# BenCooper305/RL-Cattle-Herding

Measured on AMD Instinct MI355X. Metric: env-steps/sec (agent-steps/sec) at 4096 envs/GPU, 1/2/4/8 MI355X, higher is better.
Workload: dtype f64; 1 GPU; BASELINE configs[3]: 4096 envs/GPU x (4 drones, 16 cattle), CTDE obs (12,86), random-action rollout with auto-reset; envs_per_gpu=4096, num_drones=4, num_cattle=16, mode=ctde, physics=pyb, parallelism=env-sharded x1 (no per-step collective)

## Files before the change

### rl-cattle-herding_amd/csrc/ch_api.cpp

```cpp
#include <hip/hip_runtime.h>

#include <algorithm>
#include <cstdlib>
#include <cmath>
#include <cstdio>
#include <cstring>
#include <new>
#include <string>
#include <vector>

#include "ch_handle.h"
#include "ch_spawn_table.inc"

using namespace ch;

thread_local std::string g_create_err;

static const double kEpisodeLen[8] = {40, 40, 40, 40, 80, 40, 80, 80};
static const int kLevelMin[8] = {3, 4, 4, 4, 4, 4, 4, 4};
static const int kLevelMax[8] = {3, 4, 4, 4, 4, 4, 12, 12};

static uint64_t splitmix(uint64_t& s) {
    uint64_t z = (s += 0x9E3779B97F4A7C15ull);
    z = (z ^ (z >> 30)) * 0xBF58476D1CE4E5B9ull;
// ... 657 lines not shown
}

int ch__set_geometry(ch_handle* h, int32_t G, int32_t block) {
    if (!h || G < 1 || G > 64 || G * h->NC > 64 || block < 128 || block % 64 ||
        block > ((h->pw || h->cfg.physics != CH_PHYS_PYB) ? CH_V2_MAX_BLOCK_PW : CH_V2_MAX_BLOCK))
        return CH_ERR_INVALID;
    if (G * h->M > 3 * (block - 64)) return CH_ERR_UNSUPPORTED;
    size_t lds = V2Layout(G, h->NC, h->M, h->P, h->cfg.mode, (int)h->rsize, h->pw ? block / 64 - 1 : 0).bytes();
    if (lds > 160 * 1024) return CH_ERR_UNSUPPORTED;
    bool sep = false;
    if (!h->pw) {
        const size_t l = V2Layout(G, h->NC, h->M, h->P, h->cfg.mode, (int)h->rsize, 0, true).bytes();
        if (l <= 160 * 1024) { sep = true; lds = l; }
    }
    h->G = G; h->block = block; h->lds = lds; h->sep = sep;
    HIP_TRY(h, prepare_step(h));
    return CH_OK;
}

int ch__geometry(const ch_handle* h, int32_t* G, int32_t* block, int64_t* lds, int32_t* kernel) {
    if (!h) return CH_ERR_INVALID;
    if (G) *G = h->G;
    if (block) *block = h->block;
    if (lds) *lds = (int64_t)h->lds;
    if (kernel) *kernel = h->kernel;
    return CH_OK;
}

int ch__obs_invalidate(ch_handle* h, void* stream) {
    if (!h) return CH_ERR_INVALID;
    h->obs_zero_ptr = nullptr;
    HIP_TRY(h, hipSetDevice(h->device));
    HIP_TRY(h, hipMemsetAsync(h->stale + h->E, 1, (size_t)h->E, (hipStream_t)stream));
    return CH_OK;
}

int ch__set_phase_mask(ch_handle* h, int32_t mask) {
    if (!h) return CH_ERR_INVALID;
    h->phase_mask = mask;
    return CH_OK;
}

int ch_metrics(ch_handle* h, double* out, int32_t reset_after, void* stream) {
    if (!h || !out) return fail(h, CH_ERR_INVALID, "ch_metrics: NULL argument");
    HIP_TRY(h, hipSetDevice(h->device));
    hipStream_t st = (hipStream_t)stream;
    HIP_TRY(h, launch_metrics_reduce(h->metrics, h->E, h->mdev, h->errw, h->mdev + CH_METRIC_COUNT, reset_after, st));
    HIP_TRY(h, hipMemcpyAsync(h->mhost, h->mdev, sizeof(double) * (CH_METRIC_COUNT + 1), hipMemcpyDeviceToHost, st));
    HIP_TRY(h, hipStreamSynchronize(st));
    std::memcpy(out, h->mhost, sizeof(double) * CH_METRIC_COUNT);
    return device_status(h, (int)h->mhost[CH_METRIC_COUNT]);
}

int ch_metrics_device(ch_handle* h, double* dev_out, int32_t reset_after, void* stream) {
    if (!h || !dev_out) return fail(h, CH_ERR_INVALID, "ch_metrics_device: NULL argument");
    HIP_TRY(h, hipSetDevice(h->device));
    HIP_TRY(h, launch_metrics_reduce(h->metrics, h->E, dev_out, nullptr, nullptr, reset_after, (hipStream_t)stream));
    return CH_OK;
}

int ch_get_eval(ch_handle* h, double* host_out, void* stream) {
    if (!h || !host_out) return fail(h, CH_ERR_INVALID, "ch_get_eval: NULL argument");
    if (!h->evald) return fail(h, CH_ERR_UNSUPPORTED, "ch_get_eval: the handle was created with eval_metrics = 0");
    HIP_TRY(h, hipSetDevice(h->device));
    HIP_TRY(h, hipStreamSynchronize((hipStream_t)stream));
    HIP_TRY(h, hipMemcpy(host_out, h->evald, sizeof(double) * h->E * h->NC, hipMemcpyDeviceToHost));
    return CH_OK;
}

int ch_outputs_to_host(ch_handle* h, const ch_step_io* io, ch_host_out* out, void* stream) {
    if (!h) return fail(nullptr, CH_ERR_INVALID, "ch_outputs_to_host: NULL handle");
    if (!io || !out || !io->obs || !io->reward || !io->terminated || !io->truncated || !out->obs || !out->reward ||
        !out->terminated || !out->truncated)
        return fail(h, CH_ERR_INVALID, "ch_outputs_to_host: obs, reward, terminated and truncated are required on both sides");
    if ((out->reset_happened || out->ended_env || out->ended_obs || out->ended_stats) && !io->reset_happened)
        return fail(h, CH_ERR_INVALID, "ch_outputs_to_host: the reset list needs io->reset_happened");
    if ((out->ended_obs && !io->terminal_obs) || (out->ended_stats && !io->episode_stats))
        return fail(h, CH_ERR_INVALID, "ch_outputs_to_host: ended_obs needs io->terminal_obs, ended_stats io->episode_stats");
    if (out->agent_active && !io->agent_active)
        return fail(h, CH_ERR_INVALID, "ch_outputs_to_host: agent_active needs io->agent_active");
    HIP_TRY(h, hipSetDevice(h->device));
    hipStream_t st = (hipStream_t)stream;
    const int64_t E = h->E;
    const size_t blk = (size_t)h->rows * 86, live = (size_t)h->NC * 86;
    if (io->reset_happened) {
        if (!h->st.count) {
            HIP_TRY(h, hipMalloc(&h->st.count, sizeof(long long)));
            HIP_TRY(h, hipMalloc(&h->st.env, sizeof(long long) * E));
            HIP_TRY(h, hipMalloc(&h->st.stats, sizeof(double) * 2 * E));
            HIP_TRY(h, hipMalloc(&h->st.obs, sizeof(float) * blk * E));
            HIP_TRY(h, hipHostMalloc(&h->st.count_host, sizeof(long long), hipHostMallocDefault));
        }
        HIP_TRY(h, launch_stage_ended(E, io->reset_happened, out->ended_obs ? io->terminal_obs : nullptr,
                                      out->ended_stats ? io->episode_stats : nullptr, (int)blk, h->st.count, h->st.env,
                                      h->st.stats, h->st.obs, st));
        HIP_TRY(h, hipMemcpyAsync(h->st.count_host, h->st.count, sizeof(long long), hipMemcpyDeviceToHost, st));
    }
    if (live == blk)
        HIP_TRY(h, hipMemcpyAsync(out->obs, io->obs, sizeof(float) * blk * E, hipMemcpyDeviceToHost, st));
    else
        HIP_TRY(h, hipMemcpy2DAsync(out->obs, sizeof(float) * blk, io->obs, sizeof(float) * blk, sizeof(float) * live, E,
                                    hipMemcpyDeviceToHost, st));
    const size_t K = (size_t)h->K;
    HIP_TRY(h, hipMemcpyAsync(out->reward, io->reward, sizeof(float) * K * E, hipMemcpyDeviceToHost, st));
    HIP_TRY(h, hipMemcpyAsync(out->terminated, io->terminated, K * E, hipMemcpyDeviceToHost, st));
    HIP_TRY(h, hipMemcpyAsync(out->truncated, io->truncated, K * E, hipMemcpyDeviceToHost, st));
// ... 42 lines not shown
```

### rl-cattle-herding_amd/csrc/ch_step_body.h

```cpp
#pragma once
#include <hip/hip_runtime.h>

#include <atomic>

#include "ch_common.h"
#include "ch_device.h"
#include "ch_internal.h"

namespace ch {

enum { I_N = 0, I_SC, I_SCA, I_HASPREV, I_LEVEL, I_TALLY, I_SPAWN, I_ACTIVE, I_EPISODE, I_FLOCK, I_RESET, I_NEWN,
       I_HERD, I_OBSD, I_COUNT };
static_assert(I_COUNT == kV2EnvInts, "LDS env-int rows");
enum { F_D = 0, F_T, F_H, F_A, F_E, F_R, F_X0, F_X1, F_X2,
       C_PAIRS, C_ROWS, C_COWS, C_FLOCK, C_DELTA, F_W, F_Q,
       Q_LEN, C_QUEUE, F_C,
       C_EULER,
       V_DSIMD,
       F_RSV0, F_RSV1, F_RSV2,
       F_HC,
       FLAG_COUNT };
static_assert(FLAG_COUNT <= kV2Flags, "LDS flag words");
#define FL_LIST (I_COUNT * G)
#define RS_LIST (I_COUNT * G + G)
// ... 538 lines not shown
    const R C2B = R(2 * 4.47213595499958);
    R gx = 0, gy = 0, cxx = 0, cyy = 0, sx = 0, sy = 0;
    int nb = 0;
    constexpr int NK = NT ? NT : 64;
    CH_UNROLL for (int k = 0; k < NK; ++k) {
        if (k >= N || k >= n) break;
        R t[6];
        const int f = delta_vals(S, N, u, g, k, t);
        if (f & 1) { ++nb; gx += t[0]; gy += t[1]; cxx += t[2]; cyy += t[3]; }
        if (f & 2) { sx += t[4]; sy += t[5]; }
    }
    ddx = 0; ddy = 0;
    if (nb > 0) { ddx = C2B * gx + C2B * cxx; ddy = C2B * gy + C2B * cyy; }
    ddx += sx; ddy += sy;
}

template <class R>
__device__ __forceinline__ void velocity_update(const StepParams<R>& p, const V2Smem<R>& S, int M, int e0, int u, R ddx,
                                                R ddy, R* nv = nullptr, int GM = 0) {
    const long long CS = (long long)p.E * M;
    const R C1G = R(5), C2G = R(0.2 * 2.23606797749979);
    const R qix = S.cx[u], qiy = S.cy[u], pix = S.cvx[u], piy = S.cvy[u];
    R gmx = -C1G * sigma_1(qix - R(1)) - C2G * pix, gmy = -C1G * sigma_1(qiy - R(1)) - C2G * piy;
    R qx = (S.aux[u] + ddx) + gmx, qy = (S.auy[u] + ddy) + gmy;
    const R dt_sqr = R(0.05 * 0.05);
    R vx = pix + qx * dt_sqr, vy = piy + qy * dt_sqr;
    R sp = norm2(vx, vy);
    if (sp > R(kMaxVelCattle)) { R f = R(kMaxVelCattle) / sp; vx *= f; vy *= f; }
    if (nv) { nv[u] = vx; nv[GM + u] = vy; return; }
    const long long ci = (long long)e0 * M + u;
    CH_STS(&p.cattle[2 * CS + ci], vx); CH_STS(&p.cattle[3 * CS + ci], vy);
}

template <class R>
__device__ __forceinline__ void flock_combine(const StepParams<R>& p, V2Smem<R>& S, int N, int M, int e0, int u, int n,
                                              const R* td, const uint8_t* tdf, int ib, int T) {
    const R C2B = R(2 * 4.47213595499958);
    R ddx = 0, ddy = 0, sx = 0, sy = 0, gx = 0, gy = 0, cxx = 0, cyy = 0;
    int nb = 0;
    CH_UNROLL for (int k = 0; k < N; ++k) {
        if (k >= n) break;
        const int i = ib + k;
        const int f = tdf[i];
        if (f & 1) { ++nb; gx += td[i]; gy += td[T + i]; cxx += td[2 * T + i]; cyy += td[3 * T + i]; }
        if (f & 2) { sx += td[4 * T + i]; sy += td[5 * T + i]; }
    }
    if (nb > 0) { ddx = C2B * gx + C2B * cxx; ddy = C2B * gy + C2B * cyy; }
    ddx += sx; ddy += sy;
    velocity_update(p, S, M, e0, u, ddx, ddy);
}

template <class R>
struct V2Pipe {
    enum { P_N = 0, P_B, P_C, P_SIMD, P_COUNT = 8 };
    static constexpr size_t kBytes = (27 + 7) * 64 * sizeof(R) + (2 * 64 + kV2Flags + P_COUNT) * sizeof(int);
    R *ho, *d1;
    int *hoi, *flags1, *sync;
    __device__ explicit V2Pipe(unsigned char* base) {
        ho = (R*)base; d1 = ho + 27 * 64;
        hoi = (int*)(d1 + 7 * 64); flags1 = hoi + 2 * 64; sync = flags1 + kV2Flags;
    }
};

template <class R, int MODE, int GT, int NT, int MT, bool PHYS, bool PW, bool TOBS, int ROLE = 0>
__device__ __forceinline__ void step2_body(const StepParams<R>& p, int salt = 0, int kstep = 0) {
    extern __shared__ __align__(16) unsigned char smem_[];
    unsigned char* const smem = smem_ + salt;
    constexpr bool PIPE = ROLE != 0;
    static_assert(!PIPE || (sizeof(R) == 8 && MODE == 0 && GT == 16 && NT == 4 && !PW && !TOBS && !PHYS),
                  "the pipelined step loop is the configs[3] f64 instantiation's");
    constexpr bool marl = MODE == 1;
    constexpr bool MIX = sizeof(R) == 4;
    using PT = double;
    constexpr bool QUAD = !marl && GT == 16 && NT == 4;
    const int G = GT ? GT : p.G, N = NT ? NT : p.NC, M = MT ? MT : p.M, P = MT ? MT * (MT - 1) / 2 : p.P;
    const int rows = marl ? N : 12;
    const V2Layout L(G, N, M, P, MODE, (int)sizeof(R), PW ? (int)(blockDim.x >> 6) - 1 : 0, !PW && p.sep);
    const bool sep = L.sep;
    V2Smem<R> S(smem, L);
    const int BS = (PIPE ? (int)blockDim.x - 64 : (int)blockDim.x) + salt;
    const int tid = (ROLE == 1 ? (int)(threadIdx.x & 63) : ROLE == 2 ? (int)threadIdx.x - 64 : (int)threadIdx.x) + salt;
    const bool isd = ROLE == 1 ? true : ROLE == 2 ? false : tid < 64;
    const V2Pipe<R> X(smem + (PIPE ? L.bytes() : 0));
    int* const ps = X.sync;
    int* const flags0 = S.flags;
    if constexpr (PIPE) {
        if (kstep & 1) {
            S.dx = X.d1; S.dy = S.dx + G * N; S.dz = S.dy + G * N; S.dq = S.dz + G * N;
            S.dxd = (double*)S.dx; S.dyd = (double*)S.dy;
            S.flags = X.flags1;
        }
    }
    const int e0 = (blockIdx.x + salt) * G;
    const int Gv = min(G, p.E - e0);
    const long long E = p.E, DS = E * N, CS = E * M;
    const int m_obs = M < 16 ? M : 16, cat_off = marl ? 18 : 34, RW = rows * 86;
    const bool task = !(p.phase_mask & 4);
    const int W1 = (BS >> 6) - 1;
    const int ct = tid - 64, CW = BS - 64;
    int* ei = S.ei;
    int* fl = S.flags;
    const Level* LT = S.LT;
    if (tid == 0) { TS(0, (long long)wall_clock64()); TS(2, (long long)clock64()); TS(12, (long long)__smid()); }
    if ((tid & 63) == 0 && tid < 256 && !PIPE) TS(22 + (tid >> 6), (long long)__builtin_amdgcn_s_getreg((31 << 11) | 4));

    const int nd = Gv * N;
    const bool dlane = tid < nd;
    const int dg = dlane ? tid / N : 0, dk = tid - dg * N;
    const long long di = (long long)e0 * N + tid;
    R pos[3], q[4], v[3], w[3], pid[9], ql[4], rpy_in[3] = {0, 0, 0};
    R ph_lr[4] = {0, 0, 0, 0}, ph_rr[3] = {0, 0, 0};
    int stepi = 0, n0 = 0, act0 = 0, stepi_env = 0;
    double ev_acc = 0;
    R spx_r[3] = {0, 0, 0}, spy_r[3] = {0, 0, 0};
    bool co_simd = false;
    uint8_t stale_d = 1;
    R c0[4];
    double c0d[2], prev0d;
    int ei0[10];
    R er0[2];
    double met0[kMetricRows];
    double pd[3] = {0, 0, 0};
    uint8_t stale_o = 0;
    unsigned long long tag_o = 0;
    if constexpr (PIPE) {
        if (ROLE == 1 && tid == 0) { PTS(0, (long long)clock64()); PTS(7, (long long)__builtin_amdgcn_s_getreg((31 << 11) | 4)); }
        if (ROLE == 2 && ct == 0) PTS(8, (long long)clock64());
        if (kstep > 0) {
            if (ROLE == 2) {
                lds_wait(ps + V2Pipe<R>::P_B, kstep, p.err);
                __builtin_amdgcn_fence(__ATOMIC_RELEASE, "workgroup");
                lds_signal(ps + V2Pipe<R>::P_C);
                lds_wait(ps + V2Pipe<R>::P_C, W1 * kstep, p.err);
                __builtin_amdgcn_fence(__ATOMIC_ACQUIRE, "workgroup");
                int* const flp = (kstep & 1) ? flags0 : X.flags1;
                if (ct < kV2Flags) flp[ct] = 0;
            } else {
                lds_wait(ps + V2Pipe<R>::P_N, kstep, p.err);
            }
        }
        if (ROLE == 1 && tid == 0) PTS(1, (long long)clock64());
        if (ROLE == 2 && ct == 0) PTS(9, (long long)clock64());
    }
    if (!isd) {
        if (ct < Gv * M) {
            const long long ci = (long long)e0 * M + ct;
#pragma unroll
            for (int c = 0; c < 4; ++c) c0[c] = p.cattle[c * CS + ci];
            if constexpr (MIX) { c0d[0] = p.cpos64[ci]; c0d[1] = p.cpos64[CS + ci]; }
        }
        if (ct < Gv) {
            const int e = e0 + ct;
#pragma unroll
            for (int r = 0; r < 9; ++r) ei0[r] = p.envi[r * E + e];
            stale_o = p.stale[E + e];
            tag_o = p.obs_tag[e];
            er0[0] = p.envr[e]; er0[1] = p.envr[E + e];
            if constexpr (MIX) prev0d = p.prev64[e];
#pragma unroll
            for (int r = 0; r < kMetricRows; ++r) met0[r] = p.metrics[r * E + e];
        }
    } else if (PIPE && kstep > 0) {
        const R* ho = X.ho + tid;
        pos[0] = ho[0 * 64]; pos[1] = ho[1 * 64]; pos[2] = ho[2 * 64];
#pragma unroll
        for (int c = 0; c < 4; ++c) q[c] = ho[(3 + c) * 64];
#pragma unroll
        for (int c = 0; c < 3; ++c) { v[c] = ho[(7 + c) * 64]; w[c] = ho[(10 + c) * 64]; }
#pragma unroll
        for (int c = 0; c < 9; ++c) pid[c] = ho[(13 + c) * 64];
#pragma unroll
        for (int c = 0; c < 4; ++c) ql[c] = ho[(22 + c) * 64];
        ev_acc = ho[26 * 64];
        n0 = X.hoi[tid]; stepi = X.hoi[64 + tid];
        stale_d = 1;
    } else if (dlane) {
        n0 = p.envi[0 * E + e0 + dg];
        stale_d = p.stale[e0 + dg];
        if (marl) act0 = p.envi[7 * E + e0 + dg];
        pos[0] = p.drone[0 * DS + di]; pos[1] = p.drone[1 * DS + di]; pos[2] = p.drone[2 * DS + di];
        if constexpr (MIX) {
#pragma unroll
            for (int c = 0; c < 3; ++c) { pd[c] = p.pos64[c * DS + di]; pos[c] = R(pd[c]); }
        }
#pragma unroll
        for (int c = 0; c < 4; ++c) q[c] = p.drone[(3 + c) * DS + di];
#pragma unroll
        for (int c = 0; c < 3; ++c) { v[c] = p.drone[(7 + c) * DS + di]; w[c] = p.drone[(10 + c) * DS + di]; }
#pragma unroll
        for (int c = 0; c < 9; ++c) pid[c] = p.drone[(13 + c) * DS + di];
#pragma unroll
        for (int c = 0; c < 4; ++c) ql[c] = p.drone[(22 + c) * DS + di];
#pragma unroll
        for (int c = 0; c < 3; ++c) rpy_in[c] = p.rpy[c * DS + di];
        stepi = p.envi[9 * E + e0 + dg];
        if (p.evald) ev_acc = p.evald[di];
        if constexpr (PHYS) {
#pragma unroll
            for (int c = 0; c < 4; ++c) ph_lr[c] = p.phys[c * DS + di];
#pragma unroll
            for (int c = 0; c < 3; ++c) ph_rr[c] = p.phys[(4 + c) * DS + di];
        }
    }
    if constexpr (!PIPE) {
    if (tid < Gv) stepi_env = p.envi[9 * E + e0 + tid];
    if (tid < kV2Flags) fl[tid] = 0;
    if constexpr (PW) { if (tid < G) reinterpret_cast<int*>(S.hasnb)[tid] = 0; }
    lds_barrier();
    }

    if (isd) {
        __builtin_amdgcn_s_setprio(3);
        if (tid == 0 && !PIPE)
            __hip_atomic_store(fl + V_DSIMD, 1 + (int)((__builtin_amdgcn_s_getreg((31 << 11) | 4) >> 4) & 3), __ATOMIC_RELAXED,
                               __HIP_MEMORY_SCOPE_WORKGROUP);
    } else {
        const float rM0 = 1.0f / (float)M;
        for (int u = ct; u < Gv * M; u += CW) {
            const long long ci = (long long)e0 * M + u;
            const bool first = u == ct;
            R x = first ? c0[0] : p.cattle[0 * CS + ci], y = first ? c0[1] : p.cattle[1 * CS + ci];
            const R vx = first ? c0[2] : p.cattle[2 * CS + ci], vy = first ? c0[3] : p.cattle[3 * CS + ci];
            const R dt = R(p.dt);
            double xd = 0, yd = 0;
            if constexpr (MIX) { xd = first ? c0d[0] : p.cpos64[ci]; yd = first ? c0d[1] : p.cpos64[CS + ci]; }
            if (!PHYS || (p.physics != CH_PHYS_DYN && p.physics != CH_PHYS_DYN_RK4))
                for (int s = 0; s < p.substeps; ++s) {
                    if constexpr (MIX) { xd += (double)(vx * dt); yd += (double)(vy * dt); }
                    else { x += vx * dt; y += vy * dt; }
                }
            if constexpr (MIX) {
                x = R(xd); y = R(yd);
                CH_STS(&p.cpos64[ci], xd); CH_STS(&p.cpos64[CS + ci], yd);
                S.cxd[u] = xd; S.cyd[u] = yd;
            }
            CH_STS(&p.cattle[0 * CS + ci], x); CH_STS(&p.cattle[1 * CS + ci], y);
            S.cx[u] = x; S.cy[u] = y; S.cvx[u] = vx; S.cvy[u] = vy;
        }
        for (int k = ct; k < (int)(sizeof(kLevels) / 4); k += CW)
            reinterpret_cast<uint32_t*>(S.LT)[k] = reinterpret_cast<const uint32_t*>(kLevels)[k];
        for (int k = ct; k < P; k += CW) const_cast<uint16_t*>(S.pl)[k] = p.pairs[k];
        for (int k = ct; k < G * M; k += CW) {
            S.nbm[k] = 0;
            if (sep) S.cnt[k] = 0;
        }
        if constexpr (!PW)
            for (int k = ct; k < G * P; k += CW) S.queue[k] = kQEmpty;
        if (ct < 64) {
        const int g = ct;
        bool flk = false;
        if (g < Gv) {
            const int scA = ei0[2] + 1;
            flk = (scA % 2) == 0 && !(p.phase_mask & 2);
            ei[I_N * G + g] = ei0[0]; ei[I_SC * G + g] = ei0[1]; ei[I_SCA * G + g] = scA;
            ei[I_HASPREV * G + g] = ei0[3]; ei[I_LEVEL * G + g] = ei0[4];
            ei[I_TALLY * G + g] = ei0[5]; ei[I_SPAWN * G + g] = ei0[6];
            ei[I_ACTIVE * G + g] = ei0[7]; ei[I_EPISODE * G + g] = ei0[8];
            ei[I_FLOCK * G + g] = flk; ei[I_RESET * G + g] = 0; ei[I_HERD * G + g] = 0;
            ei0[9] = stale_o | (tag_o != (unsigned long long)(uintptr_t)p.obs ? 1 : 0);
            ei[I_OBSD * G + g] = ei0[9];
            S.prev[g] = er0[0]; S.clock[g] = er0[1];
            if constexpr (MIX) S.prevd[g] = prev0d;
#pragma unroll
            for (int r = 0; r < kMetricRows; ++r) S.met[r * G + g] = met0[r];
        }
        const unsigned long long bal = __ballot(flk);
        if (flk) ei[FL_LIST + __popcll(bal & ((1ull << ct) - 1ull))] = g;
        if (ct == 0) { ei[NF_AT] = __popcll(bal); ei[NR_AT] = 0; }
        }
        cow_sync(fl + F_E, W1, false, p.err);
        {
            int ds = PIPE ? ps[V2Pipe<R>::P_SIMD + (kstep & 1)] : lds_peek(fl + V_DSIMD);
            int spins = 0;
            for (; ds == 0 && spins < (1 << 22) && !PIPE; ++spins) {
                __builtin_amdgcn_s_sleep(1);
                ds = lds_peek(fl + V_DSIMD);
            }
            spin_note(spins);
            co_simd = (int)((__builtin_amdgcn_s_getreg((31 << 11) | 4) >> 4) & 3) + 1 == ds;
        }
        if (ct == 0) TS(11, (long long)clock64());
        if (ct < 64) {
            const int g = ct;
            if (g < Gv) {
                PT sx = 0, sy = 0;
                CH_UNROLL for (int j = 0; j < M; ++j) { sx += S.cxd[g * M + j]; sy += S.cyd[g * M + j]; }
                S.hcxd[g] = sx / PT(M); S.hcyd[g] = sy / PT(M);
                if constexpr (MIX) { S.hcx[g] = R(S.hcxd[g]); S.hcy[g] = R(S.hcyd[g]); }
            }
            lds_signal(fl + F_HC);
        }
#pragma unroll
        for (int k = 0; k < 3; ++k) {
            const int u = ct + k * CW;
            if (u < Gv * M) {
                const int g = qdiv(u, M, rM0), j = u - g * M;
                int sp = ei[I_SPAWN * G + g] + 1;
                if (sp >= p.n_scen) sp = 0;
                const double* tab = p.spawn + ((long long)sp * p.n_cows + j) * 2;
                spx_r[k] = R(tab[0]); spy_r[k] = R(tab[1]);
            }
        }
    }
    if (tid == 0) TS(3, (long long)clock64());

    const bool wobs = !(p.phase_mask & 8);
    const bool late = sep && GT == 16 && NT == 4, fast = late && (TOBS || !p.terminal_obs);
    const bool tobs = TOBS && p.terminal_obs != nullptr;
    float* obs_wg = p.obs + (long long)e0 * RW;
    int f_n = 0, f_sc = 0, f_scA = 0, f_hp = 0, f_level = 0, f_tally = 0, f_spawn = 0, f_active = 0, f_episode = 0;
    PT f_prev = 0;
    R f_clock = 0;

    if (isd) {
        const int n = dlane ? n0 : 0;
        const bool live = dlane && dk < n;
        R px0 = 0, py0 = 0;
// ... 428 lines not shown
            const bool rd = dlane && ei[I_RESET * G + dg];
            const int n_new = rd ? ei[I_NEWN * G + dg] : 0;
            if (tobs && wobs && rd && live) {
                float* tb = p.terminal_obs + (long long)(e0 + dg) * RW;
                obs_own_nrpy(tb, dk, pos[2], v, w);
                if (task) obs_nbr(tb, S.dxd, S.dyd, dg * N, dk, nb1, nb2);
            }
            double xd = 0, yd = 0, zd = 0;
            if (rd) {
                reset_drone_xyz(dk, n_new, xd, yd, zd);
                S.rdx[tid] = R(xd); S.rdy[tid] = R(yd); S.rdz[tid] = R(zd);
            }
            const R z = R(zd);
            wave_sync();
            if (rd) {
                if constexpr (PIPE) {
                    R* ho = X.ho + tid;
                    ho[0 * 64] = R(xd); ho[1 * 64] = R(yd); ho[2 * 64] = R(zd);
                    ho[3 * 64] = 0; ho[4 * 64] = 0; ho[5 * 64] = 0; ho[6 * 64] = 1;
#pragma unroll
                    for (int c = 7; c < 13; ++c) ho[c * 64] = 0;
                    if (!p.compat) {
#pragma unroll
                        for (int c = 13; c < 22; ++c) ho[c * 64] = 0;
                    }
                    ho[22 * 64] = 0; ho[23 * 64] = 0; ho[24 * 64] = 0; ho[25 * 64] = 1;
                    ho[26 * 64] = 0;
                    X.hoi[tid] = n_new;
                }
                reset_drone_store(p, di, xd, yd, zd);
                if constexpr (PHYS) {
#pragma unroll
                    for (int c = 0; c < kPhysComps; ++c) CH_STS(&p.phys[c * DS + di], R(0));
                }
                CH_STS(&p.rpy[di], R(0)); CH_STS(&p.rpy[DS + di], -R(0)); CH_STS(&p.rpy[2 * DS + di], R(0));
                if (wobs) {
                    float* eb = obs_wg + dg * RW;
                    if (dk < n_new) {
                        const R zero3[3] = {0, 0, 0}, rpy0[3] = {R(0), -R(0), R(0)};
                        obs_own(eb, dk, z, rpy0, zero3, zero3);
                        const int nb = nearest_two(S.rdx, S.rdy, dg * N, dk, n_new);
                        obs_nbr(eb, S.rdx, S.rdy, dg * N, dk, (nb & 0xff) - 1, (nb >> 8) - 1);
                    } else if (dk < ei[I_N * G + dg]) {
                        for (int c = 0; c < 14; c += 2) st2(eb, dk * 86 + c, 0.0f, 0.0f);
                    }
                }
            }
        }
        if constexpr (PIPE) {
            __builtin_amdgcn_fence(__ATOMIC_RELEASE, "workgroup");
            lds_signal(ps + V2Pipe<R>::P_N);
            if (tid == 0) PTS(5, (long long)clock64());
        }
        R qpb[NQ], qsa[NQ], qsb[NQ], qca[NQ], qcb[NQ], qps[NQ], qsc[NQ];
        if constexpr (!marl) {
            if (live && task) {
                if constexpr (QUAD) q_sc = cattle_term(S, tid, M, R(p.cs_cc));
                else S.scat[tid] = cattle_term(S, tid, M, R(p.cs_cc));
            }
            if constexpr (QUAD) {
                qall(q_pa, qpa); qall(q_pb, qpb);
                qall(q_sa, qsa); qall(q_sb, qsb); qall(q_ca, qca); qall(q_cb, qcb); qall(q_ps, qps); qall(q_sc, qsc);
            } else {
                wave_sync();
            }
        }
        if (envl && task) {
            const int n = f_n;
            if constexpr (!marl) {
                const Level& Lv = LT[level_r];
                R sp_simple = 0, sp_complex = 0, msp = 0, mcat = 0, cat = 0;
                R psp_i[NT ? NT : 12], scat_i[NT ? NT : 12];
                CH_UNROLL for (int i = 0; i < N; ++i) {
                    const bool li = i < n;
                    const int iq = i % NQ;
                    const R pa = QUAD ? qpa[iq] : S.pa[b0 + i], pb = QUAD ? qpb[iq] : S.pb[b0 + i];
                    const bool ua = li && (p.compat || pa < R(INFINITY)), ub = li && (p.compat || pb < R(INFINITY));
                    sp_complex += ua ? (QUAD ? qca[iq] : S.ca[b0 + i]) : R(0);
                    sp_simple += ua ? (QUAD ? qsa[iq] : S.sa[b0 + i]) : R(0);
                    sp_complex += ub ? (QUAD ? qcb[iq] : S.cb[b0 + i]) : R(0);
                    sp_simple += ub ? (QUAD ? qsb[iq] : S.sb[b0 + i]) : R(0);
                    psp_i[i] = QUAD ? qps[iq] : S.psp[b0 + i]; scat_i[i] = QUAD ? qsc[iq] : S.scat[b0 + i];
                }
                const R n2 = R(n * 2.0), nn = R(n);
                sp_complex = divc(sp_complex, n2); sp_simple = divc(sp_simple, n2);
                R approach = 0;
                if (f_hp) approach = R(clip(divc(f_prev - cent, max_step_p + PT(1e-6)) * PT(5), PT(-1.0), PT(1.0)));
                f_prev = cent; f_hp = 1;
                CH_UNROLL for (int i = 0; i < N; ++i) cat += i < n ? scat_i[i] : R(0);
                cat = divc(cat, nn);
                R rg = sp_simple * R(Lv.w_simple) + sp_complex * R(Lv.w_complex) + R(0.1) * R(Lv.w_survival) +
                       approach * R(Lv.w_approach) + divc(eff, R(100)) * R(Lv.w_eff) + cat * R(Lv.w_cattle);
                CH_UNROLL for (int i = 0; i < N; ++i) { msp += i < n ? psp_i[i] : R(0); mcat += i < n ? scat_i[i] : R(0); }
                msp = divc(msp, nn); mcat = divc(mcat, nn);
                R tot = 0;
                CH_UNROLL for (int i = 0; i < N; ++i) tot += i < n ? rg + R(0.5) * ((psp_i[i] - msp) + (scat_i[i] - mcat)) : R(0);
                R rew = divc(tot, nn);
                if (envw) {
                    CH_ST(&p.reward[e], (float)rew);
                    p.term[e] = te2; p.trunc[e] = tr;
                }
                ret = (double)rew;
                n_term = te2; n_trunc = tr; n_nan = rew != rew;
            }
            if (g == 0) TS(19, (long long)clock64());
            f_sc += marl ? 1 : p.substeps;
            const double* mt = S.met;
            double o[kMetricRows];
#pragma unroll
            for (int r = 0; r < kMetricRows; ++r) o[r] = mt[r * G + g];
            o[CH_METRIC_STEPS] += 1;
            o[CH_METRIC_TERMINATED] += n_term;
            o[CH_METRIC_TRUNCATED] += n_trunc;
            o[CH_METRIC_NAN_REWARDS] += n_nan;
            o[CH_METRIC_EFFECTIVENESS_SUM] += (double)eff;
            o[kMetricCurReturn] += ret;
            o[kMetricCurLen] += 1;
            if (done) {
                if (p.episode_stats && envw) {
                    CH_ST(&p.episode_stats[2 * (long long)e], o[kMetricCurReturn]);
                    CH_ST(&p.episode_stats[2 * (long long)e + 1], o[kMetricCurLen]);
                }
                o[CH_METRIC_EPISODES] += 1;
                o[CH_METRIC_RETURN_SUM] += o[kMetricCurReturn];
                o[CH_METRIC_LENGTH_SUM] += o[kMetricCurLen];
                o[kMetricCurReturn] = 0;
                o[kMetricCurLen] = 0;
            }
#pragma unroll
            for (int r = 0; r < kMetricRows; ++r)
                if (envw) CH_STS(&p.metrics[r * E + e], o[r]);
            if (g == 0) TS(28, (long long)clock64());
            if (p.reset_happened && envw) p.reset_happened[e] = rs;
            if (rs) reset_scalars(p, e, f_n, f_sc, f_scA, f_spawn, f_episode, f_active, f_hp, f_prev, f_clock, n_next);
            if (p.agent_active && envw)
                for (int i = 0; i < N; ++i) p.agent_active[(long long)e * N + i] = (f_active >> i) & 1;
        } else if (envw && p.reset_happened) {
            p.reset_happened[e] = 0;
        }
        if (tid == 0) TS(7, (long long)clock64());
        if (QUAD ? envw : tid < Gv) {
            const int e = e0 + (QUAD ? dg : tid);
            CH_STS(&p.envi[0 * E + e], f_n); CH_STS(&p.envi[1 * E + e], f_sc); CH_STS(&p.envi[2 * E + e], f_scA);
            CH_STS(&p.envi[3 * E + e], f_hp); CH_STS(&p.envi[4 * E + e], f_level); CH_STS(&p.envi[5 * E + e], f_tally);
            CH_STS(&p.envi[6 * E + e], f_spawn); CH_STS(&p.envi[7 * E + e], f_active); CH_STS(&p.envi[8 * E + e], f_episode);
            CH_STS(&p.envi[9 * E + e], (QUAD ? stepi : stepi_env) + 1);
            CH_STS(&p.envr[0 * E + e], R(f_prev)); CH_STS(&p.envr[1 * E + e], f_clock);
            if constexpr (MIX) CH_STS(&p.prev64[e], f_prev);
            p.stale[e] = 0;
            if (wobs) p.stale[E + e] = 0;
            p.obs_tag[e] = wobs ? (unsigned long long)(uintptr_t)p.obs : 0ull;
        }
        if constexpr (PIPE) {
            __builtin_amdgcn_fence(__ATOMIC_RELEASE, "workgroup");
            lds_signal(ps + V2Pipe<R>::P_B);
            if (tid == 0) PTS(6, (long long)clock64());
        }
    } else {
        const float rM = 1.0f / (float)M;
        const int nf = ei[NF_AT];
        const int* flist = ei + FL_LIST;
        const int lane = tid & 63;
        const bool co = co_simd && W1 >= 4;
        const bool skip_pre = co && (PW ? (p.phase_mask & 256) != 0 : !(p.phase_mask & 256));
        const bool skip_post = co && (p.phase_mask & 128);
        bool skip_now = skip_pre;
        R* tb = nullptr;
        uint8_t* tf = nullptr;
        uint16_t* qu = nullptr;
        int f_cur = -1, ch = 0, qn = 0, qd = 0;
        const int NCH = (P + 63) >> 6;
        constexpr int NCHC = MT > 0 ? (MT * (MT - 1) / 2 + 63) / 64 : 1;
        uint32_t prw[NCHC];
#pragma unroll
        for (int c = 0; c < NCHC; ++c) {
            const int r = 64 * c + (tid & 63);
            prw[c] = (PW && MT > 0) ? S.pl[r < P ? r : 0] : 0u;
        }
        R* const nv = S.td + 2 * G * M;
        auto spawn_d = [&](int g, int j, int c) -> double {
            int sp = ei[I_SPAWN * G + g] + 1;
            if (sp >= p.n_scen) sp = 0;
            return p.spawn[((long long)sp * p.n_cows + j) * 2 + c];
        };
        auto store_final = [&](int u) {
            const int g = qdiv(u, M, 1.0f / (float)M);
            const long long ci = (long long)e0 * M + u;
            R vx = nv[u], vy = nv[G * M + u];
            if (fast && ei[I_RESET * G + g])
                reset_cow_vel(p, ci, p.env_off + e0 + g, u - g * M, (uint32_t)ei[I_EPISODE * G + g], vx, vy);
            CH_STS(&p.cattle[2 * CS + ci], vx); CH_STS(&p.cattle[3 * CS + ci], vy);
        };
        auto arrive = [&](int u) {
            __builtin_amdgcn_fence(__ATOMIC_RELEASE, "workgroup", "local");
            const int old = __hip_atomic_fetch_add(&S.cnt[u], 1, __ATOMIC_RELAXED, __HIP_MEMORY_SCOPE_WORKGROUP);
            if ((old & 3) == 1) {
                __builtin_amdgcn_fence(__ATOMIC_ACQUIRE, "workgroup", "local");
                if (!late) {
                    velocity_update(p, S, M, e0, u, S.td[u], S.td[G * M + u]);
                } else {
                    velocity_update(p, S, M, e0, u, S.td[u], S.td[G * M + u], nv, G * M);
                    __builtin_amdgcn_fence(__ATOMIC_RELEASE, "workgroup", "local");
                    const int o2 = __hip_atomic_fetch_add(&S.cnt[u], 8, __ATOMIC_RELAXED, __HIP_MEMORY_SCOPE_WORKGROUP);
                    if (o2 & 4) store_final(u);
                }
            }
        };
        auto arrive_final = [&](int u) {
            __builtin_amdgcn_fence(__ATOMIC_RELEASE, "workgroup", "local");
// ... 25 lines not shown
                for (int j = lane; j < M; j += 64) alpha_row_pw(S, M, P, g, j, tb);
                wave_sync();
                if constexpr (PW) lds_signal(reinterpret_cast<int*>(S.hasnb) + f_cur);
                f_cur = -1;
            }
            CHUNK_T1(0);
            return true;
        };
        if constexpr (PW) {
            tb = S.tgx + (size_t)(tid / 64 - 1) * L.slot;
            tf = S.tdf + (size_t)(tid / 64 - 1) * M * N;
            qu = S.queue + (size_t)(tid / 64 - 1) * P;
        } else {
            alpha_cheap(S, fl, M, P, nf, flist, skip_pre);
            if (ct == 0) TS(38, (long long)clock64());
            lds_signal(fl + F_C);
            if (ct == 0) { TS(39, (long long)clock64()); TS(29, (long long)lds_peek(fl + Q_LEN)); }
            alpha_full(S, fl, M, P, skip_pre, W1, p.err);
        }
        if (ct == 0) TS(18, (long long)clock64());
#pragma unroll
        for (int k = 0; k < 3; ++k) {
            const int u = ct + k * CW;
            if (u < Gv * M) { S.spx[u] = spx_r[k]; S.spy[u] = spy_r[k]; }
        }
        if (wobs)
            for (int g = 0; g < Gv; ++g)
                if (p.obs_full || ei[I_OBSD * G + g]) obs_zero_env(obs_wg + g * RW, ei[I_N * G + g], rows, cat_off, m_obs, ct, CW);
        if constexpr (PW) {
            while (lds_peek(fl + F_D) < 1 && alpha_step()) {
            }
        } else {
            lds_signal(fl + F_A);
            int sleeps = 0;
            for (int spins = 0; spins < (1 << 22); ++spins) {
                if (lds_peek(fl + F_D) >= 1) break;
                if (lds_peek(fl + F_A) < W1) { __builtin_amdgcn_s_sleep(1); ++sleeps; continue; }
                __builtin_amdgcn_fence(__ATOMIC_ACQUIRE, "workgroup", "local");
                const int b = grab(fl + C_ROWS, 64, skip_pre), u = b + lane;
                if (b >= nf * M) break;
                CHUNK_T0;
                if (u < nf * M) {
                    const int f = qdiv(u, M, rM), g = flist[f], j = u - f * M;
                    alpha_row(S, M, P, g * M + j, g, j);
                    if (sep) arrive(g * M + j);
                }
                CHUNK_T1(2);
            }
            spin_note(sleeps);
        }
        if (ct == 0) { TS(8, (long long)clock64()); PTS(10, (long long)clock64()); }
        lds_wait(fl + F_D, 1, p.err);
        if (ct == 0) { TS(9, (long long)clock64()); PTS(11, (long long)clock64()); }
        skip_now = skip_post;
        for (;;) {
            const int b = grab(fl + C_COWS, 64, skip_post), u = b + lane;
            if (b >= Gv * M) break;
            CHUNK_T0;
            if (u < Gv * M) {
            const int g = qdiv(u, M, rM), j = u - g * M;
            const int n = ei[I_N * G + g], b0 = g * N;
            const R qix = S.cx[u], qiy = S.cy[u];
            CH_UNROLL for (int k = 0; k < N; ++k) {
                if (k >= n) break;
                const R ex = S.dx[b0 + k] - qix, ey = S.dy[b0 + k] - qiy;
                S.dcow[(b0 + k) * M + j] = ex * ex + ey * ey;
            }
            if (task) {
                int wn = 0;
                CH_UNROLL for (int i = 0; i < N; ++i) {
                    if (i >= n) break;
                    int i2 = (i + 1 == n) ? 0 : i + 1;
                    R x1 = S.dx[b0 + i], y1 = S.dy[b0 + i], x2 = S.dx[b0 + i2], y2 = S.dy[b0 + i2];
                    R il = (x2 - x1) * (qiy - y1) - (qix - x1) * (y2 - y1);
                    if (y1 <= qiy) { if (y2 > qiy && il > R(0)) wn += 1; }
                    else { if (y2 <= qiy && il < R(0)) wn -= 1; }
                }
                if (wn != 0) atomicAdd(&ei[I_HERD * G + g], 1);
            }
            if (j < m_obs && wobs && !late) obs_cattle(obs_wg + g * RW, S.dxd, S.dyd, b0, j, n, cat_off, S.cxd[u], S.cyd[u]);
            }
            __builtin_amdgcn_fence(__ATOMIC_RELEASE, "workgroup", "local");
            if (lane == 0) __hip_atomic_fetch_add(fl + F_H, min(64, Gv * M - b), __ATOMIC_RELAXED, __HIP_MEMORY_SCOPE_WORKGROUP);
            CHUNK_T1(1);
        }
        const float rN = 1.0f / (float)N;
        auto euler_pass = [&]() {
          for (;;) {
            const int b = grab(fl + C_EULER, 64, skip_post), t = b + lane;
            if (b >= 3 * Gv * N) break;
            if (t < 3 * Gv * N) {
                const int c = t >= Gv * N ? (t >= 2 * Gv * N ? 2 : 1) : 0, u = t - c * Gv * N;
                const int g = qdiv(u, N, rN), k = u - g * N;
                const bool rsf = fast && ei[I_RESET * G + g];
                if (k < ei[I_N * G + g] && (!rsf || (tobs && wobs))) {
                    const int GN = G * N;
                    const R qq[4] = {S.dq[u], S.dq[GN + u], S.dq[2 * GN + u], S.dq[3 * GN + u]};
                    const R r = quat_to_euler_c(qq, c);
                    const long long dd = (long long)e0 * N + u;
                    if (!rsf) {
                        CH_STS(&p.rpy[c * DS + dd], r);
                        if (wobs) CH_ST(obs_wg + g * RW + k * 86 + 1 + c, (float)r);
                    } else {
                        CH_ST(p.terminal_obs + (long long)(e0 + g) * RW + k * 86 + 1 + c, (float)r);
                    }
                }
// ... 193 lines not shown
                if (ct >= c0l && u < nr * M) {
                    const int k0 = qdiv(u, M, rM), g = rl[k0], j = u - k0 * M, uc = g * M + j;
                    reset_cow_vel(p, (long long)e0 * M + uc, p.env_off + e0 + g, j, (uint32_t)ei[I_EPISODE * G + g],
                                  cvx_r[i], cvy_r[i]);
                }
            }
            if (ct == 0) TS(55, (long long)clock64());
            cow_sync(fl + F_X1, W1, true, p.err);
            if (ct == 0) TS(53, (long long)clock64());
            if (dit) {
                const int k0 = qdiv(ct, N, rN), g = rl[k0], k = ct - k0 * N, ud = g * N + k;
                const int n = ei[I_NEWN * G + g];
                const long long dd = (long long)e0 * N + ud;
                reset_drone_store(p, dd, rx, ry, rz);
                if constexpr (PHYS) {
#pragma unroll
                    for (int c = 0; c < kPhysComps; ++c) CH_STS(&p.phys[c * DS + dd], R(0));
                }
                CH_STS(&p.rpy[dd], R(0)); CH_STS(&p.rpy[DS + dd], -R(0)); CH_STS(&p.rpy[2 * DS + dd], R(0));
                if (wobs) {
                    float* eb = obs_wg + g * RW;
                    if (k < n) {
                        const R zero3[3] = {0, 0, 0}, rpy0[3] = {R(0), -R(0), R(0)};
                        obs_own(eb, k, R(rz), rpy0, zero3, zero3);
                        const int nb = nearest_two(S.rdx, S.rdy, g * N, k, n);
                        obs_nbr(eb, S.rdx, S.rdy, g * N, k, (nb & 0xff) - 1, (nb >> 8) - 1);
                    } else if (k < ei[I_N * G + g]) {
                        for (int c = 0; c < 86; c += 2) st2(eb, k * 86 + c, 0.0f, 0.0f);
                    }
                }
            }
            if (ct >= c0l)
                for (int u = ct - c0l, i = 0; u < nr * M; u += cl, ++i) {
                    const int k0 = qdiv(u, M, rM), g = rl[k0], j = u - k0 * M, uc = g * M + j;
                    R vx = i == 0 ? cvx_r[0] : cvx_r[1], vy = i == 0 ? cvy_r[0] : cvy_r[1];
                    if (i >= RI)
                        reset_cow_vel(p, (long long)e0 * M + uc, p.env_off + e0 + g, j, (uint32_t)ei[I_EPISODE * G + g], vx, vy);
                    const double x = MIX ? spawn_d(g, j, 0) : (double)S.spx[uc], y = MIX ? spawn_d(g, j, 1) : (double)S.spy[uc];
                    reset_cow_store(p, (long long)e0 * M + uc, x, y, vx, vy);
                    if (wobs && j < m_obs) obs_cattle(obs_wg + g * RW, S.rdx, S.rdy, g * N, j, ei[I_NEWN * G + g], cat_off, x, y);
                }
            if (ct == 0) TS(54, (long long)clock64());
        }
    }
    if (tid == 0) TS(35, (long long)clock64());
    if (tid == 64) TS(36, (long long)clock64());
    if (tid >= 64) { TS_MAX(63); PTS_MAX(15); }
    if (p.tstamp) {
        if constexpr (!PIPE) lds_barrier();
        if (tid == 0) { TS(13, (long long)clock64()); TS(14, (long long)clock64()); TS(1, (long long)wall_clock64()); }
    }
}


template <class R, int MODE, int GT, int NT, int MT>
__device__ __forceinline__ void step2_pipe_init(const StepParams<R>& p) {
    extern __shared__ __align__(16) unsigned char smem_[];
    const V2Layout L(GT, NT, MT, MT * (MT - 1) / 2, MODE, (int)sizeof(R), 0, p.sep != 0);
    V2Smem<R> S(smem_, L);
    const V2Pipe<R> X(smem_ + L.bytes());
    const int t = threadIdx.x;
    if (t < kV2Flags) { S.flags[t] = 0; X.flags1[t] = 0; }
    if (t < V2Pipe<R>::P_SIMD) X.sync[t] = 0;
    if ((t & 63) == 0 && t < 128)
        X.sync[V2Pipe<R>::P_SIMD + (t >> 6)] = 1 + (int)((__builtin_amdgcn_s_getreg((31 << 11) | 4) >> 4) & 3);
    lds_barrier();
}

}
```

Before: 308.6 million env-steps/s.

## Signal env write-back earlier in pipelined step and keep metrics in LDS across steps

In the pipelined f64 step loop, the per-env scalar update and global write-back now happen before the reward/metric computation, so the next step's producer is signalled (P_B) earlier. A new P_K counter guards the later consumers. Per-env metric rows now stay in a dedicated LDS area across steps instead of being reloaded from global memory each step. The level table and pair list are loaded once at pipe init rather than every step. The cost is a larger LDS footprint, extra synchronisation, and reordering that has to keep the old prev/hp values correct for the reward.

```diff
diff --git a/rl-cattle-herding_amd/csrc/ch_api.cpp b/rl-cattle-herding_amd/csrc/ch_api.cpp
--- a/rl-cattle-herding_amd/csrc/ch_api.cpp
+++ b/rl-cattle-herding_amd/csrc/ch_api.cpp
@@ -733,6 +733,15 @@
     return device_status(h, (int)h->mhost[CH_METRIC_COUNT]);
 }
 
+int ch__metric_rows(ch_handle* h, double* host_out, void* stream) {
+    if (!h || !host_out) return fail(h, CH_ERR_INVALID, "ch__metric_rows: NULL argument");
+    HIP_TRY(h, hipSetDevice(h->device));
+    hipStream_t st = (hipStream_t)stream;
+    HIP_TRY(h, hipMemcpyAsync(host_out, h->metrics, sizeof(double) * kMetricRows * h->E, hipMemcpyDeviceToHost, st));
+    HIP_TRY(h, hipStreamSynchronize(st));
+    return CH_OK;
+}
+
 int ch_metrics_device(ch_handle* h, double* dev_out, int32_t reset_after, void* stream) {
     if (!h || !dev_out) return fail(h, CH_ERR_INVALID, "ch_metrics_device: NULL argument");
     HIP_TRY(h, hipSetDevice(h->device));
diff --git a/rl-cattle-herding_amd/csrc/ch_step_body.h b/rl-cattle-herding_amd/csrc/ch_step_body.h
--- a/rl-cattle-herding_amd/csrc/ch_step_body.h
+++ b/rl-cattle-herding_amd/csrc/ch_step_body.h
@@ -614,15 +614,36 @@
 
 template <class R>
 struct V2Pipe {
-    enum { P_N = 0, P_B, P_C, P_SIMD, P_COUNT = 8 };
-    static constexpr size_t kBytes = (27 + 7) * 64 * sizeof(R) + (2 * 64 + kV2Flags + P_COUNT) * sizeof(int);
+    enum { P_N = 0, P_B, P_C, P_SIMD, P_K = P_SIMD + 2, P_COUNT = 8 };
+    static_assert(P_K < P_COUNT, "launch-long counters");
+    static constexpr int kMetG = 16;
+    static constexpr size_t kBytes = (27 + 7) * 64 * sizeof(R) + (size_t)kMetricRows * kMetG * sizeof(double) +
+                                     (2 * 64 + kV2Flags + P_COUNT) * sizeof(int);
     R *ho, *d1;
+    double* met;
     int *hoi, *flags1, *sync;
     __device__ explicit V2Pipe(unsigned char* base) {
         ho = (R*)base; d1 = ho + 27 * 64;
-        hoi = (int*)(d1 + 7 * 64); flags1 = hoi + 2 * 64; sync = flags1 + kV2Flags;
+        met = (double*)(d1 + 7 * 64);
+        hoi = (int*)(met + kMetricRows * kMetG); flags1 = hoi + 2 * 64; sync = flags1 + kV2Flags;
     }
 };
+
+#define CH_ENV_WRITE_BACK() do { \
+        if (QUAD ? envw : tid < Gv) {                                                                                    \
+            const int e = e0 + (QUAD ? dg : tid);                                                                        \
+            CH_STS(&p.envi[0 * E + e], f_n); CH_STS(&p.envi[1 * E + e], f_sc); CH_STS(&p.envi[2 * E + e], f_scA);        \
+            CH_STS(&p.envi[3 * E + e], f_hp); CH_STS(&p.envi[4 * E + e], f_level); CH_STS(&p.envi[5 * E + e], f_tally);  \
+            CH_STS(&p.envi[6 * E + e], f_spawn); CH_STS(&p.envi[7 * E + e], f_active); CH_STS(&p.envi[8 * E + e], f_episode); \
+            CH_STS(&p.envi[9 * E + e], (QUAD ? stepi : stepi_env) + 1);                       \
+            CH_STS(&p.envr[0 * E + e], R(f_prev)); CH_STS(&p.envr[1 * E + e], f_clock);                                  \
+            if constexpr (MIX) CH_STS(&p.prev64[e], f_prev);                                                             \
+                             \
+            p.stale[e] = 0;                                                                                              \
+            if (wobs) p.stale[E + e] = 0;                                                                                \
+            p.obs_tag[e] = wobs ? (unsigned long long)(uintptr_t)p.obs : 0ull;                                           \
+        }                                                                                                                \
+    } while (0)
 
 template <class R, int MODE, int GT, int NT, int MT, bool PHYS, bool PW, bool TOBS, int ROLE = 0>
 __device__ __forceinline__ void step2_body(const StepParams<R>& p, int salt = 0, int kstep = 0) {
@@ -631,6 +652,7 @@
     constexpr bool PIPE = ROLE != 0;
     static_assert(!PIPE || (sizeof(R) == 8 && MODE == 0 && GT == 16 && NT == 4 && !PW && !TOBS && !PHYS),
                   "the pipelined step loop is the configs[3] f64 instantiation's");
+    static_assert(!PIPE || GT == V2Pipe<R>::kMetG, "X.met holds kMetG envs per metric row");
     constexpr bool marl = MODE == 1;
     constexpr bool MIX = sizeof(R) == 4;
     using PT = double;
@@ -686,7 +708,7 @@
     uint8_t stale_o = 0;
     unsigned long long tag_o = 0;
     if constexpr (PIPE) {
-        if (ROLE == 1 && tid == 0) { PTS(0, (long long)clock64()); PTS(7, (long long)__builtin_amdgcn_s_getreg((31 << 11) | 4)); }
+        if (ROLE == 1 && tid == 0) PTS(0, (long long)clock64());
         if (ROLE == 2 && ct == 0) PTS(8, (long long)clock64());
         if (kstep > 0) {
             if (ROLE == 2) {
@@ -719,8 +741,10 @@
             tag_o = p.obs_tag[e];
             er0[0] = p.envr[e]; er0[1] = p.envr[E + e];
             if constexpr (MIX) prev0d = p.prev64[e];
-#pragma unroll
-            for (int r = 0; r < kMetricRows; ++r) met0[r] = p.metrics[r * E + e];
+            if (!PIPE || kstep == 0) {
+#pragma unroll
+                for (int r = 0; r < kMetricRows; ++r) met0[r] = p.metrics[r * E + e];
+            }
         }
     } else if (PIPE && kstep > 0) {
         const R* ho = X.ho + tid;
@@ -799,9 +823,11 @@
             CH_STS(&p.cattle[0 * CS + ci], x); CH_STS(&p.cattle[1 * CS + ci], y);
             S.cx[u] = x; S.cy[u] = y; S.cvx[u] = vx; S.cvy[u] = vy;
         }
-        for (int k = ct; k < (int)(sizeof(kLevels) / 4); k += CW)
-            reinterpret_cast<uint32_t*>(S.LT)[k] = reinterpret_cast<const uint32_t*>(kLevels)[k];
-        for (int k = ct; k < P; k += CW) const_cast<uint16_t*>(S.pl)[k] = p.pairs[k];
+        if constexpr (!PIPE) {
+            for (int k = ct; k < (int)(sizeof(kLevels) / 4); k += CW)
+                reinterpret_cast<uint32_t*>(S.LT)[k] = reinterpret_cast<const uint32_t*>(kLevels)[k];
+            for (int k = ct; k < P; k += CW) const_cast<uint16_t*>(S.pl)[k] = p.pairs[k];
+        }
         for (int k = ct; k < G * M; k += CW) {
             S.nbm[k] = 0;
             if (sep) S.cnt[k] = 0;
@@ -823,8 +849,15 @@
             ei[I_OBSD * G + g] = ei0[9];
             S.prev[g] = er0[0]; S.clock[g] = er0[1];
             if constexpr (MIX) S.prevd[g] = prev0d;
-#pragma unroll
-            for (int r = 0; r < kMetricRows; ++r) S.met[r * G + g] = met0[r];
+            if constexpr (PIPE) {
+                if (kstep == 0) {
+#pragma unroll
+                    for (int r = 0; r < kMetricRows; ++r) X.met[r * G + g] = met0[r];
+                }
+            } else {
+#pragma unroll
+                for (int r = 0; r < kMetricRows; ++r) S.met[r * G + g] = met0[r];
+            }
         }
         const unsigned long long bal = __ballot(flk);
         if (flk) ei[FL_LIST + __popcll(bal & ((1ull << ct) - 1ull))] = g;
@@ -1359,6 +1392,20 @@
             lds_signal(ps + V2Pipe<R>::P_N);
             if (tid == 0) PTS(5, (long long)clock64());
         }
+        int r_n = 0, r_hp = 0;
+        PT r_prev = 0;
+        if constexpr (PIPE) { r_n = f_n; r_hp = f_hp; r_prev = f_prev; }
+        if constexpr (PIPE) {
+            if (envl && task) {
+                f_prev = cent; f_hp = 1;
+                f_sc += p.substeps;
+                if (rs) reset_scalars(p, e, f_n, f_sc, f_scA, f_spawn, f_episode, f_active, f_hp, f_prev, f_clock, n_next);
+            }
+            CH_ENV_WRITE_BACK();
+            __builtin_amdgcn_fence(__ATOMIC_RELEASE, "workgroup");
+            lds_signal(ps + V2Pipe<R>::P_B);
+            if (tid == 0) PTS(6, (long long)clock64());
+        }
         R qpb[NQ], qsa[NQ], qsb[NQ], qca[NQ], qcb[NQ], qps[NQ], qsc[NQ];
         if constexpr (!marl) {
             if (live && task) {
@@ -1372,8 +1419,14 @@
                 wave_sync();
             }
         }
+        if constexpr (PIPE) {
+            if (kstep > 0) {
+                lds_wait(ps + V2Pipe<R>::P_K, kstep, p.err);
+                __builtin_amdgcn_fence(__ATOMIC_ACQUIRE, "workgroup");
+            }
+        }
         if (envl && task) {
-            const int n = f_n;
+            const int n = PIPE ? r_n : f_n;
             if constexpr (!marl) {
                 const Level& Lv = LT[level_r];
                 R sp_simple = 0, sp_complex = 0, msp = 0, mcat = 0, cat = 0;
@@ -1392,8 +1445,9 @@
                 const R n2 = R(n * 2.0), nn = R(n);
                 sp_complex = divc(sp_complex, n2); sp_simple = divc(sp_simple, n2);
                 R approach = 0;
-                if (f_hp) approach = R(clip(divc(f_prev - cent, max_step_p + PT(1e-6)) * PT(5), PT(-1.0), PT(1.0)));
-                f_prev = cent; f_hp = 1;
+                if (PIPE ? r_hp : f_hp)
+                    approach = R(clip(divc((PIPE ? r_prev : f_prev) - cent, max_step_p + PT(1e-6)) * PT(5), PT(-1.0), PT(1.0)));
+                if constexpr (!PIPE) { f_prev = cent; f_hp = 1; }
                 CH_UNROLL for (int i = 0; i < N; ++i) cat += i < n ? scat_i[i] : R(0);
                 cat = divc(cat, nn);
                 R rg = sp_simple * R(Lv.w_simple) + sp_complex * R(Lv.w_complex) + R(0.1) * R(Lv.w_survival) +
@@ -1411,8 +1465,9 @@
                 n_term = te2; n_trunc = tr; n_nan = rew != rew;
             }
             if (g == 0) TS(19, (long long)clock64());
-            f_sc += marl ? 1 : p.substeps;
-            const double* mt = S.met;
+            if constexpr (!PIPE) f_sc += marl ? 1 : p.substeps;
+            double* mt = S.met;
+            if constexpr (PIPE) mt = X.met;
             double o[kMetricRows];
 #pragma unroll
             for (int r = 0; r < kMetricRows; ++r) o[r] = mt[r * G + g];
@@ -1436,32 +1491,29 @@
             }
 #pragma unroll
             for (int r = 0; r < kMetricRows; ++r)
-                if (envw) CH_STS(&p.metrics[r * E + e], o[r]);
+                if (envw) {
+                    CH_STS(&p.metrics[r * E + e], o[r]);
+                    if constexpr (PIPE) mt[r * G + g] = o[r];
+                }
             if (g == 0) TS(28, (long long)clock64());
             if (p.reset_happened && envw) p.reset_happened[e] = rs;
-            if (rs) reset_scalars(p, e, f_n, f_sc, f_scA, f_spawn, f_episode, f_active, f_hp, f_prev, f_clock, n_next);
+            if constexpr (!PIPE) {
+                if (rs) reset_scalars(p, e, f_n, f_sc, f_scA, f_spawn, f_episode, f_active, f_hp, f_prev, f_clock, n_next);
+            }
             if (p.agent_active && envw)
                 for (int i = 0; i < N; ++i) p.agent_active[(long long)e * N + i] = (f_active >> i) & 1;
         } else if (envw && p.reset_happened) {
             p.reset_happened[e] = 0;
         }
         if (tid == 0) TS(7, (long long)clock64());
-        if (QUAD ? envw : tid < Gv) {
-            const int e = e0 + (QUAD ? dg : tid);
-            CH_STS(&p.envi[0 * E + e], f_n); CH_STS(&p.envi[1 * E + e], f_sc); CH_STS(&p.envi[2 * E + e], f_scA);
-            CH_STS(&p.envi[3 * E + e], f_hp); CH_STS(&p.envi[4 * E + e], f_level); CH_STS(&p.envi[5 * E + e], f_tally);
-            CH_STS(&p.envi[6 * E + e], f_spawn); CH_STS(&p.envi[7 * E + e], f_active); CH_STS(&p.envi[8 * E + e], f_episode);
-            CH_STS(&p.envi[9 * E + e], (QUAD ? stepi : stepi_env) + 1);
-            CH_STS(&p.envr[0 * E + e], R(f_prev)); CH_STS(&p.envr[1 * E + e], f_clock);
-            if constexpr (MIX) CH_STS(&p.prev64[e], f_prev);
-            p.stale[e] = 0;
-            if (wobs) p.stale[E + e] = 0;
-            p.obs_tag[e] = wobs ? (unsigned long long)(uintptr_t)p.obs : 0ull;
-        }
         if constexpr (PIPE) {
             __builtin_amdgcn_fence(__ATOMIC_RELEASE, "workgroup");
-            lds_signal(ps + V2Pipe<R>::P_B);
-            if (tid == 0) PTS(6, (long long)clock64());
+            lds_signal(ps + V2Pipe<R>::P_K);
+            if (tid == 0)
+                PTS(7, (long long)((unsigned long long)clock64() & ((1ull << 62) - 1)) |
+                           (long long)((unsigned long long)((__builtin_amdgcn_s_getreg((31 << 11) | 4) >> 4) & 3) << 62));
+        } else {
+            CH_ENV_WRITE_BACK();
         }
     } else {
         const float rM = 1.0f / (float)M;
@@ -1593,6 +1645,12 @@
         if (ct == 0) { TS(8, (long long)clock64()); PTS(10, (long long)clock64()); }
         lds_wait(fl + F_D, 1, p.err);
         if (ct == 0) { TS(9, (long long)clock64()); PTS(11, (long long)clock64()); }
+        if constexpr (PIPE) {
+            if (kstep > 0) {
+                lds_wait(ps + V2Pipe<R>::P_K, kstep, p.err);
+                __builtin_amdgcn_fence(__ATOMIC_ACQUIRE, "workgroup");
+            }
+        }
         skip_now = skip_post;
         for (;;) {
             const int b = grab(fl + C_COWS, 64, skip_post), u = b + lane;
@@ -1892,6 +1950,7 @@
     }
 }
 
+#undef CH_ENV_WRITE_BACK
 
 template <class R, int MODE, int GT, int NT, int MT>
 __device__ __forceinline__ void step2_pipe_init(const StepParams<R>& p) {
@@ -1901,9 +1960,12 @@
     const V2Pipe<R> X(smem_ + L.bytes());
     const int t = threadIdx.x;
     if (t < kV2Flags) { S.flags[t] = 0; X.flags1[t] = 0; }
-    if (t < V2Pipe<R>::P_SIMD) X.sync[t] = 0;
+    if (t < V2Pipe<R>::P_SIMD || t == V2Pipe<R>::P_K) X.sync[t] = 0;
     if ((t & 63) == 0 && t < 128)
         X.sync[V2Pipe<R>::P_SIMD + (t >> 6)] = 1 + (int)((__builtin_amdgcn_s_getreg((31 << 11) | 4) >> 4) & 3);
+    for (int k = t; k < (int)(sizeof(kLevels) / 4); k += (int)blockDim.x)
+        reinterpret_cast<uint32_t*>(S.LT)[k] = reinterpret_cast<const uint32_t*>(kLevels)[k];
+    for (int k = t; k < MT * (MT - 1) / 2; k += (int)blockDim.x) const_cast<uint16_t*>(S.pl)[k] = p.pairs[k];
     lds_barrier();
 }
 
```

New measurement: 319.9 million env-steps/s (median of 6 runs). +3.7%, better.
